# aghasemzadeh/OpenMPL

Hardware: AMD Instinct MI355X
Metric: poses/sec (V=4, J=17, batch=1024 per GPU) fp32 (higher is better)
Workload: dtype f32; 1 GPU; Human3.6M config: V=4 J=17 batch=1024 fp32, CHOSEN flag set, depth 12, DIM 32, heads 8; global_batch=1024, parallelism=single GPU

## Files before the change

openmpl_amd/csrc/spt_native.hip:

```cpp
#include <type_traits>

#include "spt_stage.hpp"

namespace mpl {

constexpr int QS = 100;
constexpr int SPT_LDS_BYTES = (ROWS * XS + ROWS * QS) * 4;

__device__ __forceinline__ int spt_abl(const SptParams& p) {
#ifdef MPL_LAB
    return p.abl;
#else
    return 0;
#endif
}

__device__ __forceinline__ void ln_frags(const float* X, int m, int li, int kq, const float4& g0, const float4& g1,
                                         const float4& b0, const float4& b1, float4& a0, float4& a1) {
    const float* xr = X + (m * 16 + li) * XS + 4 * kq;
    float4 x0 = ld4(xr), x1 = ld4(xr + 16);
    float s = ((x0.x + x0.y) + (x0.z + x0.w)) + ((x1.x + x1.y) + (x1.z + x1.w));
    s = xor16_add(s);
    s = xor32_add(s);
    const float mean = s * (1.0f / 32.0f);
    x0.x -= mean; x0.y -= mean; x0.z -= mean; x0.w -= mean;
    x1.x -= mean; x1.y -= mean; x1.z -= mean; x1.w -= mean;
    float ss = ((x0.x * x0.x + x0.y * x0.y) + (x0.z * x0.z + x0.w * x0.w)) +
               ((x1.x * x1.x + x1.y * x1.y) + (x1.z * x1.z + x1.w * x1.w));
    ss = xor16_add(ss);
    ss = xor32_add(ss);
    const float rstd = 1.0f / sqrtf(ss * (1.0f / 32.0f) + 1e-6f);
    a0.x = x0.x * rstd * g0.x + b0.x; a0.y = x0.y * rstd * g0.y + b0.y;
    a0.z = x0.z * rstd * g0.z + b0.z; a0.w = x0.w * rstd * g0.w + b0.w;
    a1.x = x1.x * rstd * g1.x + b1.x; a1.y = x1.y * rstd * g1.y + b1.y;
    a1.z = x1.z * rstd * g1.z + b1.z; a1.w = x1.w * rstd * g1.w + b1.w;
}

struct BlockFrags {
    float4 wq[6][2]; float bq[6];
    float4 wp[2][2]; float bp[2];
    float4 w1[4][2]; float b1[4];
    float4 w2[2][4]; float b2[2];
    float4 g1a, g1b, e1a, e1b;
    float4 g2a, g2b, e2a, e2b;
};

template <int N, int K>
__device__ __forceinline__ void load_tiles(const float* w, const float* b, int ldw, float4 (&wf)[N][K], float (&bf)[N], int li, int kq) {
#pragma unroll
    for (int n = 0; n < N; ++n) {
        const gfp wr = G(w) + (n * 16 + li) * ldw + 4 * kq;
#pragma unroll
        for (int q = 0; q < K; ++q) wf[n][q] = ld4(wr + 16 * q);
        bf[n] = G(b)[n * 16 + li];
    }
}
__device__ __forceinline__ void load_ln(const float* w, const float* b, float4& g0, float4& g1, float4& e0, float4& e1, int kq) {
    g0 = ld4(G(w) + 4 * kq); g1 = ld4(G(w) + 16 + 4 * kq);
    e0 = ld4(G(b) + 4 * kq); e1 = ld4(G(b) + 16 + 4 * kq);
}

constexpr int SPT_WB_VEC = 8192;
constexpr int SPT_WB_FLOATS = SPT_WB_VEC + 512;
constexpr int SPT_SMALL_ROWS = 144;
constexpr int SPT_SMALL_LDS_BYTES = (SPT_SMALL_ROWS * (XS + QS) + 2 * SPT_WB_FLOATS) * 4;
__device__ __forceinline__ const float* spt_uniform(const float* q) {
    const unsigned long long v = (unsigned long long)(uintptr_t)q;
    const unsigned lo = __builtin_amdgcn_readfirstlane((unsigned)v), hi = __builtin_amdgcn_readfirstlane((unsigned)(v >> 32));
    return reinterpret_cast<const float*>((uintptr_t)(((unsigned long long)hi << 32) | lo));
}
__device__ __forceinline__ void stage_block(const mpl_block_weights& bwv, float* wb, int wave, int lane, int w0, int nw) {
    if (wave < w0 || wave >= w0 + nw) return;
    const int li = lane & 15, kq = lane >> 4;
    struct { const float *qkv_w, *proj_w, *fc1_w, *fc2_w, *qkv_b, *proj_b, *fc1_b, *fc2_b, *ln1_w, *ln1_b, *ln2_w, *ln2_b; } bw;
    bw.qkv_w = spt_uniform(bwv.qkv_w); bw.proj_w = spt_uniform(bwv.proj_w); bw.fc1_w = spt_uniform(bwv.fc1_w); bw.fc2_w = spt_uniform(bwv.fc2_w);
    bw.qkv_b = spt_uniform(bwv.qkv_b); bw.proj_b = spt_uniform(bwv.proj_b); bw.fc1_b = spt_uniform(bwv.fc1_b); bw.fc2_b = spt_uniform(bwv.fc2_b);
    bw.ln1_w = spt_uniform(bwv.ln1_w); bw.ln1_b = spt_uniform(bwv.ln1_b); bw.ln2_w = spt_uniform(bwv.ln2_w); bw.ln2_b = spt_uniform(bwv.ln2_b);
    const unsigned lds0 = __builtin_amdgcn_readfirstlane((unsigned)(uintptr_t)(__attribute__((address_space(3))) float*)wb);
    for (int pc = wave - w0; pc < 34; pc += nw) {
        const float* src;
        bool on = true;
        if (pc < 12) src = bw.qkv_w + ((pc >> 1) * 16 + li) * SD + 16 * (pc & 1) + 4 * kq;
        else if (pc < 16) src = bw.proj_w + (((pc - 12) >> 1) * 16 + li) * SD + 16 * (pc & 1) + 4 * kq;
        else if (pc < 24) src = bw.fc1_w + (((pc - 16) >> 1) * 16 + li) * SD + 16 * (pc & 1) + 4 * kq;
        else if (pc < 32) src = bw.fc2_w + (((pc - 24) >> 2) * 16 + li) * (2 * SD) + 16 * (pc & 3) + 4 * kq;
        else if (pc == 32)
            src = lane < 24 ? bw.qkv_b + 4 * lane
                : lane < 32 ? bw.proj_b + 4 * (lane - 24)
                : lane < 48 ? bw.fc1_b + 4 * (lane - 32)
                : lane < 56 ? bw.fc2_b + 4 * (lane - 48) : bw.ln1_w + 4 * (lane - 56);
        else {
            src = lane < 8 ? bw.ln1_b + 4 * lane : lane < 16 ? bw.ln2_w + 4 * (lane - 8) : bw.ln2_b + 4 * (lane - 16);
            on = lane < 24;
        }
        if (on) dma16(src, lds0 + (unsigned)(pc * 1024));
    }
}
__device__ __forceinline__ float4 wb4(const float* wb, int piece, int lane) { return *reinterpret_cast<const float4*>(wb + piece * 256 + lane * 4); }
__device__ __forceinline__ float4 wbv4(const float* wb, int off, int kq) { return *reinterpret_cast<const float4*>(wb + SPT_WB_VEC + off + 4 * kq); }

__device__ __forceinline__ void touch(const float4& a) {
    const f32x4 v = {a.x, a.y, a.z, a.w};
    asm volatile("" ::"v"(v));
}
__device__ __forceinline__ void touch(float a) { asm volatile("" ::"v"(a)); }

__device__ __forceinline__ f32x4 tile_k32(const float4& a0, const float4& a1, const float4& w0, const float4& w1) {
    f32x4 c0 = f32x4{0.f, 0.f, 0.f, 0.f}, c1 = c0;
    c0 = mfma16(a0.x, w0.x, c0); c1 = mfma16(a1.x, w1.x, c1);
    c0 = mfma16(a0.y, w0.y, c0); c1 = mfma16(a1.y, w1.y, c1);
    c0 = mfma16(a0.z, w0.z, c0); c1 = mfma16(a1.z, w1.z, c1);
    c0 = mfma16(a0.w, w0.w, c0); c1 = mfma16(a1.w, w1.w, c1);
    return c0 + c1;
}

enum { P_QKV = 0, P_PROJ = 1, P_FC1 = 2, P_FC2 = 3 };
template <int P>
struct Phase {
    static constexpr int NT = P == P_QKV ? 6 : P == P_FC1 ? 4 : 2;
    static constexpr int KH = P == P_FC2 ? 4 : 2;
    static constexpr int PIECE = P == P_QKV ? 0 : P == P_PROJ ? 12 : P == P_FC1 ? 16 : 24;
    static constexpr int BIAS = P == P_QKV ? 0 : P == P_PROJ ? 96 : P == P_FC1 ? 128 : 192;
    static constexpr int LN = P == P_QKV ? 224 : 288;
// ... 58 lines not shown
    __device__ __forceinline__ void begin(const mpl_block_weights&, const mpl_block_weights&, bool) {}
};

template <int P, class Weights, class AFrags, class Epilogue>
__device__ __forceinline__ void linear_phase(const Weights& W, int mt, int wave, bool skip, AFrags a_frags, Epilogue epilogue) {
    constexpr int NT = Phase<P>::NT, KH = Phase<P>::KH;
    const int lo = (mt * NT * wave) / NWAVE, hi = (mt * NT * (wave + 1)) / NWAVE;
    for (int m = lo / NT; m * NT < hi && !skip; ++m) {
        float4 a[KH];
        a_frags(m, a);
#pragma unroll
        for (int n = 0; n < NT; ++n) {
            const int u = m * NT + n;
            if (u < lo || u >= hi) continue;
            float4 w[KH];
            float bias;
            W.template tile<P>(n, w, bias);
            f32x4 c = tile_k32(a[0], a[1], w[0], w[1]);
            if constexpr (KH == 4) c = c + tile_k32(a[2], a[3], w[2], w[3]);
            epilogue(m, n, c, bias);
        }
    }
}

template <bool STAGED>
__global__ __launch_bounds__(NTHR, 1) void spt_kernel(const SptParams p) {
    extern __shared__ __attribute__((aligned(1024))) float smem[];
    constexpr int RX = STAGED ? SPT_SMALL_ROWS : ROWS;
    float* WB = smem;
    float* X = smem + (STAGED ? 2 * SPT_WB_FLOATS : 0);
    float* Q = X + RX * XS;

    const int tid = threadIdx.x, lane = tid & 63, wave = __builtin_amdgcn_readfirstlane(tid >> 6);
    const int li = lane & 15, kq = lane >> 4;
    const int view = blockIdx.x % p.V;
    const int b0 = (blockIdx.x / p.V) * p.spw;
    const mpl_spt_set set = p.sets[(p.flags & MPL_F_MULTI_SPT) ? view : 0];
    const float *pose = p.poses[view], *ray = p.rays[view], *cen = p.centers[view];
    const int nl = p.B - b0 < p.spw ? p.B - b0 : p.spw;
    const int rows_live = nl * SJ;
    const int mt = (rows_live + 15) >> 4;

    std::conditional_t<STAGED, StagedWeights, FragWeights> W;
    W.li = li, W.kq = kq;
    if constexpr (STAGED) W.lane = lane;
    mpl_block_weights bw, bw_next;
    if (p.n_apps > 0) {
        bw = set.blocks[p.sched[0] & 0x7f];
        if constexpr (STAGED) stage_block(bw, WB, wave, lane, 0, NWAVE);
        else W.template load<P_QKV>(bw);
        if (STAGED && p.n_apps > 1) bw_next = set.blocks[p.sched[1] & 0x7f];
    }

    spt_embed<false>(p, set, X, tid, b0, pose, ray, cen, nl, mt * 16);
    unsigned char* sched_l = reinterpret_cast<unsigned char*>(WB + SPT_WB_FLOATS + SPT_WB_VEC + 352);
    float* conf_l = WB + SPT_WB_VEC + 352;
    if (STAGED) {
        if (tid < MPL_MAX_APPS) sched_l[tid] = p.sched[tid];
        for (int r = tid; r < rows_live; r += NTHR) {
            const int sq = r / SJ;
            conf_l[r] = pose[((size_t)(b0 + sq) * SJ + (r - sq * SJ)) * 3 + 2];
        }
        asm volatile("s_waitcnt vmcnt(0)" ::: "memory");
    }
    __syncthreads();

    const int abl = spt_abl(p);
    const bool no_mfma = (abl & 4) != 0;
    unsigned long long ph[6] = {0, 0, 0, 0, 0, 0}, tlast = (abl & 16) ? __builtin_amdgcn_s_memtime() : 0;
    auto stamp = [&](int k) {
        if (abl & 16) { const unsigned long long now = __builtin_amdgcn_s_memtime(); ph[k] += now - tlast; tlast = now; }
    };
    float4 g[2], e[2];
    auto a_ln = [&](int m, float4 (&a)[2]) { ln_frags(X, m, li, kq, g[0], g[1], e[0], e[1], a[0], a[1]); };
    auto a_q = [&](int m, auto& a) {
        const float* ar = Q + (m * 16 + li) * QS + 4 * kq;
#pragma unroll
        for (int q = 0; q < (int)(sizeof(a) / sizeof(a[0])); ++q) a[q] = ld4(ar + 16 * q);
    };
    auto add_to_x = [&](int m, int n, const f32x4& c, float b) {
        float* xd = X + (m * 16 + 4 * kq) * XS + n * 16 + li;
#pragma unroll
        for (int r = 0; r < 4; ++r) xd[r * XS] += c[r] + b;
    };
    for (int app = 0; app < p.n_apps; ++app) {
        const bool weighted = ((STAGED ? sched_l[app] : p.sched[app]) & 0x80) != 0;
        const bool more = app + 1 < p.n_apps;
        if (!STAGED && more) bw_next = set.blocks[p.sched[app + 1] & 0x7f];
        if constexpr (STAGED) W.wb = WB + (app & 1) * SPT_WB_FLOATS;
        mpl_block_weights bw_after;

        W.template begin<P_QKV>(bw, bw_next, more);
        W.template ln<P_QKV>(g, e);
        linear_phase<P_QKV>(W, mt, wave, no_mfma, a_ln, [&](int m, int n, const f32x4& c, float b) {
            float* qd = Q + (m * 16 + 4 * kq) * QS + n * 16 + li;
#pragma unroll
            for (int r = 0; r < 4; ++r) qd[r * QS] = c[r] + b;
        });
        __syncthreads();
        stamp(0);

        if (STAGED && more) {
            const int busy = (rows_live * SH + 63) >> 6;
            const int w0 = busy < NWAVE - 1 ? busy : 0;
            stage_block(bw_next, WB + ((app + 1) & 1) * SPT_WB_FLOATS, wave, lane, w0, NWAVE - w0);
            if (app + 2 < p.n_apps) bw_after = set.blocks[sched_l[app + 2] & 0x7f];
        }
// ... 19 lines not shown
            }
            float inv = 1.0f / l;
            if (weighted) {
                const int b = b0 + sq;
                if (STAGED) inv *= conf_l[r];
                else inv *= (b < p.B) ? pose[((size_t)b * SJ + (r - sq * SJ)) * 3 + 2] : 0.f;
            }
            float4 o = {0.f, 0.f, 0.f, 0.f};
#pragma unroll
            for (int j = 0; j < SJ; ++j) {
                const float4 v = ld4(kb + j * QS + SD);
                const float pj = sc[j] * inv;
                o.x = fmaf(pj, v.x, o.x);
                o.y = fmaf(pj, v.y, o.y);
                o.z = fmaf(pj, v.z, o.z);
                o.w = fmaf(pj, v.w, o.w);
            }
            st4(Q + r * QS + 4 * h, o);
        }
        __syncthreads();
        stamp(1);

        W.template begin<P_PROJ>(bw, bw_next, more);
        linear_phase<P_PROJ>(W, mt, wave, no_mfma, a_q, add_to_x);
        __syncthreads();
        stamp(2);

        W.template begin<P_FC1>(bw, bw_next, more);
        W.template ln<P_FC1>(g, e);
        linear_phase<P_FC1>(W, mt, wave, no_mfma, a_ln, [&](int m, int n, const f32x4& c, float b) {
            float* qd = Q + (m * 16 + 4 * kq) * QS + n * 16 + li;
#pragma unroll
            for (int r = 0; r < 4; ++r) qd[r * QS] = (abl & 2) ? (c[r] + b) : gelu_erf(c[r] + b);
        });
        __syncthreads();
        stamp(3);

        W.template begin<P_FC2>(bw, bw_next, more);
        linear_phase<P_FC2>(W, mt, wave, no_mfma, a_q, add_to_x);
        if (STAGED) asm volatile("s_waitcnt vmcnt(0)" ::: "memory");
        __syncthreads();
        stamp(4);
        bw = bw_next;
        if (STAGED && app + 2 < p.n_apps) bw_next = bw_after;
    }

    if (abl & 16) {
        if (lane == 0 && blockIdx.x < 32) {
            float* o = p.xs + (size_t)(blockIdx.x * NWAVE + wave) * 8;
            for (int k = 0; k < 6; ++k) o[k] = (float)ph[k];
        }
        return;
    }
    spt_epilogue<false>(p, X, tid, view, b0, pose, ray, cen, nl, rows_live);
}

int launch_spt_native(const SptParams& p, int form, int grid, hipStream_t s) {
    if (form == MPL_SPT_STAGED) {
        if (int rc = kernel_lds_once<spt_kernel<true>>(SPT_SMALL_LDS_BYTES)) return rc;
        hipLaunchKernelGGL(spt_kernel<true>, dim3(grid), dim3(NTHR), SPT_SMALL_LDS_BYTES, s, p);
    } else {
        if (int rc = kernel_lds_once<spt_kernel<false>>(SPT_LDS_BYTES)) return rc;
        hipLaunchKernelGGL(spt_kernel<false>, dim3(grid), dim3(NTHR), SPT_LDS_BYTES, s, p);
    }
    return hip_check_launch();
}

}
```

openmpl_amd/csrc/spt_packed.hip:

```cpp
#include "spt_pack.hpp"
#include "spt_stage.hpp"

namespace mpl {

constexpr int ATS = 36;
constexpr int HS = 68;
constexpr int KV_F = SJ * SH * SEQ * 4;
constexpr int SPT3_RING_BYTES = (ROWS * XS + 2 * KV_F + ROWS * ATS) * 4;
constexpr int SPT3_LDS_BYTES = 160 * 1024;
constexpr int SPT3_HID_OFF = 3072;
constexpr int SPT3_Q_OFF = 20480;
static_assert(SPT3_HID_OFF + ROWS * HS <= 2 * KV_F + ROWS * ATS, "HID does not fit its alias");
static_assert((SPT3_HID_OFF + ROWS * HS - 2 * KV_F) * 4 <= SPT3_Q_OFF, "HID reaches into the staged qkv weights");
static_assert(SPT3_Q_OFF + 12 * 1024 <= ROWS * ATS * 4, "staged qkv weights do not fit behind HID in ATT");
static_assert(SPT3_RING_BYTES + 8 * 1024 + 2 * SPT3_NPAR * 4 <= SPT3_LDS_BYTES, "spare LDS too small");

typedef float f32x2 __attribute__((ext_vector_type(2)));

__device__ inline float spt_window_scale(float v) {
    if (!(v > 0.f) || !(v < 3.0e38f)) return 1.0f;
    int e;
    (void)frexpf(32768.0f / v, &e);
    e = e - 1 < -100 ? -100 : (e - 1 > 100 ? 100 : e - 1);
    return ldexpf(1.0f, e);
}

__global__ __launch_bounds__(256) void spt_pack_kernel(const float* __restrict__ qkv_w, const float* __restrict__ qkv_b,
                                                        const float* __restrict__ ln1_w, const float* __restrict__ ln1_b,
                                                        const float* __restrict__ proj_w, const float* __restrict__ proj_b,
                                                        const float* __restrict__ fc1_w, const float* __restrict__ fc1_b,
                                                        const float* __restrict__ ln2_w, const float* __restrict__ ln2_b,
                                                        const float* __restrict__ fc2_w, const float* __restrict__ fc2_b,
                                                        char* __restrict__ dst, int fold_q) {
    __shared__ float Wf[8192];
    __shared__ float cn[SPT_NCOL], sw[SPT_NCOL], bnd[SPT_NCOL], scal[2];
    const int tid = threadIdx.x;
    for (int i = tid; i < 8192; i += 256) {
        float w;
        if (i < 3072) w = qkv_w[i] * ln1_w[i & 31];
        else if (i < 4096) w = proj_w[i - 3072];
        else if (i < 6144) w = fc1_w[i - 4096] * ln2_w[i & 31];
        else w = fc2_w[i - 6144];
        Wf[i] = w;
    }
    __syncthreads();
    if (tid < SPT_NCOL) {
        const int n = tid;
        const float *wr, *raw, *beta = nullptr;
        int K = 32;
        float bias;
        if (n < 96) { wr = Wf + n * 32; raw = qkv_w + n * 32; beta = ln1_b; bias = qkv_b[n]; }
        else if (n < 128) { wr = Wf + 3072 + (n - 96) * 32; raw = proj_w + (n - 96) * 32; bias = proj_b[n - 96]; }
        else if (n < 192) { wr = Wf + 4096 + (n - 128) * 32; raw = fc1_w + (n - 128) * 32; beta = ln2_b; bias = fc1_b[n - 128]; }
        else { wr = Wf + 6144 + (n - 192) * 64; raw = fc2_w + (n - 192) * 64; bias = fc2_b[n - 192]; K = 64; }
        float amax = 0.f;
        double ss = 0.0, c = (double)bias;
        for (int k = 0; k < K; ++k) {
            amax = fmaxf(amax, fabsf(wr[k]));
            ss += (double)wr[k] * (double)wr[k];
            if (beta) c += (double)raw[k] * (double)beta[k];
        }
        float s = 1.0f;
        if (amax > 0.f && amax < 3.0e38f) {
            int e;
            (void)frexpf(amax, &e);
            e = 14 - e;
            e = e < -100 ? -100 : (e > 100 ? 100 : e);
            s = ldexpf(1.0f, e);
// ... 136 lines not shown
#define SPT_ROLE(W, MTS, KS, LN, GELU, NCT, AST, DST, ...) \
    spt_linear_role<KS, LN, GELU, NCT, AST, DST, ((MTS) * (NCT) * (W)) / NWAVE, ((MTS) * (NCT) * ((W) + 1)) / NWAVE>(__VA_ARGS__)
#define SPT_BY_WAVE(wv, ...)                          \
    switch (wv) {                                     \
        case 0: SPT_ROLE(0, __VA_ARGS__); break;      \
        case 1: SPT_ROLE(1, __VA_ARGS__); break;      \
        case 2: SPT_ROLE(2, __VA_ARGS__); break;      \
        case 3: SPT_ROLE(3, __VA_ARGS__); break;      \
        case 4: SPT_ROLE(4, __VA_ARGS__); break;      \
        case 5: SPT_ROLE(5, __VA_ARGS__); break;      \
        case 6: SPT_ROLE(6, __VA_ARGS__); break;      \
        default: SPT_ROLE(7, __VA_ARGS__); break;     \
    }


template <int SS>
__global__ __launch_bounds__(NTHR, 1) void spt3_kernel(const SptParams p) {
    constexpr int RLIVE = SJ * SS;
    constexpr int MTS = (RLIVE + 15) / 16;
    constexpr int NT = (MTS + 3) / 4;
    extern __shared__ __attribute__((aligned(16))) float smem[];
    float* X = smem;
    float* Kb = smem + ROWS * XS;
    float* Vb = Kb + KV_F;
    float* ATT = Vb + KV_F;
    float* HID = Kb + SPT3_HID_OFF;
    char* S_W = reinterpret_cast<char*>(ATT + ROWS * ATS);
    float* S_PAR = reinterpret_cast<float*>(S_W + 8 * 1024);
    char* R_F1 = reinterpret_cast<char*>(Kb);
    char* R_Q = reinterpret_cast<char*>(ATT) + SPT3_Q_OFF;

    const int tid = threadIdx.x, lane = tid & 63;
    const int wave = __builtin_amdgcn_readfirstlane(tid >> 6);
    const int li = lane & 15, kq = lane >> 4;
    auto phase_sync = [&]() {
        asm volatile("s_waitcnt vmcnt(0)" ::: "memory");
        __syncthreads();
    };
    const int hg = wave & 1, part = wave >> 1;
    const int view = blockIdx.x % p.V;
    const int b0 = (blockIdx.x / p.V) * SS;
    const int sl = li % SS;
    const mpl_spt_set set = p.sets[(p.flags & MPL_F_MULTI_SPT) ? view : 0];
    const float* pose = p.poses[view];
    const float* ray = p.rays[view];
    const float* cen = p.centers[view];

    auto stage_w = [&](char* dst, const unsigned short* pack, int byte_off, int n_pieces) {
        const unsigned l0 = (unsigned)(uintptr_t)(__attribute__((address_space(3))) char*)dst;
        for (int i = wave; i < n_pieces; i += NWAVE)
            ::mpl::dma16(reinterpret_cast<const float*>(reinterpret_cast<const char*>(pack) + byte_off + i * 1024) + lane * 4,
                         l0 + (unsigned)(i * 1024));
    };
    auto load_par = [&](const mpl_block_weights& b) -> float4 {
        if (tid >= SPT3_NPAR / 4) return float4{0.f, 0.f, 0.f, 0.f};
        return ld4(G(reinterpret_cast<const float*>(reinterpret_cast<const char*>(b.qkv_w3) + SPT_PACK_VEC)) + 4 * tid);
    };
    auto store_par = [&](int app_of, const float4& v) {
        if (tid < SPT3_NPAR / 4) st4(S_PAR + (app_of & 1) * SPT3_NPAR + 4 * tid, v);
    };
    mpl_block_weights bw;
    if (p.n_apps > 0) {
        bw = set.blocks[p.sched[0] & 0x7f];
        stage_w(R_Q, bw.qkv_w3, SPT_PACK_QKV, 12);
    }
    const float4 par0 = p.n_apps > 0 ? load_par(bw) : float4{0.f, 0.f, 0.f, 0.f};
    spt_embed<true, SS>(p, set, X, tid, b0, pose, ray, cen, SS, MTS * 16);
    store_par(0, par0);
    phase_sync();

    auto load_w = [&](const char* region, int unit, sf16x8 (&w)[2]) { spt_load_unit(region, unit, lane, w); };
    auto ln_frag = [&](int m, sf16x8& ah, sf16x8& al) {
        const float* xr = X + (m * 16 + li) * XS + 8 * kq;
        spt_ln_split(::mpl::ld4(xr), ::mpl::ld4(xr + 4), ah, al);
    };
    for (int app = 0; app < p.n_apps; ++app) {
        const bool weighted = (p.sched[app] & 0x80) != 0;
        bw = set.blocks[p.sched[app] & 0x7f];
        const unsigned short* pack = bw.qkv_w3;
        const float* par = S_PAR + (app & 1) * SPT3_NPAR;
        stage_w(S_W, pack, SPT_PACK_PROJ, 4);
        {
            sf16x8 wq[3][2];
            float4 bq[3], sq[3];
#pragma unroll
            for (int c = 0; c < 3; ++c) {
                load_w(R_Q, 2 * c + hg, wq[c]);
                bq[c] = ::mpl::ld4(par + SPT_C_QKV + 32 * c + 16 * hg + 4 * kq);
                sq[c] = ::mpl::ld4(par + SPT_NCOL + SPT_C_QKV + 32 * c + 16 * hg + 4 * kq);
            }
            float4 q[NT];
#pragma unroll
            for (int t = 0; t < NT; ++t) {
                q[t] = float4{0.f, 0.f, 0.f, 0.f};
                if (part + 4 * t < MTS && !(p.abl & 8)) {
                    const int m = part + 4 * t;
                    const int j = (16 * m + li) / SS;
                    const bool live = 16 * m + li < RLIVE;
                    sf16x8 ah, al;
                    ln_frag(m, ah, al);
                    const f32x4 z = {0.f, 0.f, 0.f, 0.f};
                    const f32x4 cq = mfma3(wq[0], ah, al, z), ck = mfma3(wq[1], ah, al, z), cv = mfma3(wq[2], ah, al, z);
                    q[t] = float4{fmaf(cq[0], sq[0].x, bq[0].x), fmaf(cq[1], sq[0].y, bq[0].y), fmaf(cq[2], sq[0].z, bq[0].z),
                                  fmaf(cq[3], sq[0].w, bq[0].w)};
                    const int h = 4 * hg + kq;
                    const float kx = fmaf(ck[0], sq[1].x, bq[1].x), ky = fmaf(ck[1], sq[1].y, bq[1].y);
                    const float kz = fmaf(ck[2], sq[1].z, bq[1].z), kw = fmaf(ck[3], sq[1].w, bq[1].w);
                    if (live && j < SJ - 1) {
                        float* kp = Kb + ((((j >> 1) * 2) * SH + h) * SS + sl) * 4 + (j & 1);
                        kp[0] = kx;
                        kp[2] = ky;
                        kp[SH * SS * 4] = kz;
                        kp[SH * SS * 4 + 2] = kw;
                    } else if (live) {
                        st4(Kb + (SJ - 1) * SH * SS * 4 + (h * SS + sl) * 4, float4{kx, ky, kz, kw});
                    }
                    if (live)
                        st4(Vb + ((j * SH + h) * SS + sl) * 4, float4{fmaf(cv[0], sq[2].x, bq[2].x), fmaf(cv[1], sq[2].y, bq[2].y),
                                                                       fmaf(cv[2], sq[2].z, bq[2].z), fmaf(cv[3], sq[2].w, bq[2].w)});
                }
// ... 55 lines not shown
                for (int t = 0; t < NL; ++t) o[t] = float4{0.f, 0.f, 0.f, 0.f};
#pragma unroll
                for (int j = 0; j < SJ; ++j) {
                    const float4 v = ::mpl::ld4(Vb + ((j * SH + h) * SS + sl) * 4);
#pragma unroll
                    for (int t = 0; t < NL; ++t) {
                        const float pj = sc[t][j];
                        o[t].x = fmaf(pj, v.x, o[t].x);
                        o[t].y = fmaf(pj, v.y, o[t].y);
                        o[t].z = fmaf(pj, v.z, o[t].z);
                        o[t].w = fmaf(pj, v.w, o[t].w);
                    }
                }
#pragma unroll
                for (int t = 0; t < NL; ++t) {
                    o[t] = float4{o[t].x * inv[t], o[t].y * inv[t], o[t].z * inv[t], o[t].w * inv[t]};
                    if (weighted) {
                        const float big = fmaxf(fmaxf(fabsf(o[t].x), fabsf(o[t].y)), fmaxf(fabsf(o[t].z), fabsf(o[t].w)));
                        if (!(big <= 65000.f)) {
                            const float qn = __builtin_nanf("");
                            o[t] = float4{qn, qn, qn, qn};
                            if (p.err_host) __hip_atomic_fetch_or(p.err_host, 2u, __ATOMIC_RELAXED, __HIP_MEMORY_SCOPE_SYSTEM);
                        }
                    }
                }
#pragma unroll
                for (int t = 0; t < NL; ++t) st4(ATT + ((part + 4 * t) * 16 + li) * ATS + 4 * h, o[t]);
            };
            if (!(p.abl & 1)) {
                if (part + 4 * (NT - 1) < MTS) attention(SptInt<NT>{});
                else if (NT > 1) attention(SptInt<(NT > 1 ? NT - 1 : 1)>{});
            }
        }
        phase_sync();
        stage_w(R_F1, pack, SPT_PACK_FC1, 8);
        if (!(p.abl & 32)) SPT_BY_WAVE(wave, MTS, 1, false, false, 2, ATS, XS, ATT, X, S_W, par, SPT_C_PROJ, 0.f, lane);
        phase_sync();
        stage_w(S_W, pack, SPT_PACK_FC2, 8);
        if (!(p.abl & 64))
            SPT_BY_WAVE(wave, MTS, 1, true, true, 4, XS, HS, X, HID, R_F1, par, SPT_C_FC1, par[2 * SPT_NCOL + 1], lane);
        phase_sync();
        {
            float4 parn = float4{0.f, 0.f, 0.f, 0.f};
            if (app + 1 < p.n_apps) {
                const mpl_block_weights bn = set.blocks[p.sched[app + 1] & 0x7f];
                stage_w(R_Q, bn.qkv_w3, SPT_PACK_QKV, 12);
                parn = load_par(bn);
            }
            if (!(p.abl & 128)) SPT_BY_WAVE(wave, MTS, 2, false, false, 2, HS, XS, HID, X, S_W, par, SPT_C_FC2, 0.f, lane);
            if (app + 1 < p.n_apps) store_par(app + 1, parn);
        }
        phase_sync();
    }
    spt_epilogue<true, SS>(p, X, tid, view, b0, pose, ray, cen, SS, MTS * 16);
}

template <int SS>
static int launch_spt3(const SptParams& p, int grid, hipStream_t s) {
    if (int rc = kernel_lds_once<spt3_kernel<SS>>(SPT3_LDS_BYTES)) return rc;
    hipLaunchKernelGGL(spt3_kernel<SS>, dim3(grid), dim3(NTHR), SPT3_LDS_BYTES, s, p);
    return hip_check_launch();
}

int launch_spt_packed(const SptParams& p, int ss, int grid, hipStream_t s) {
    switch (ss) {
        case 1: return launch_spt3<1>(p, grid, s);
        case 2: return launch_spt3<2>(p, grid, s);
        case 4: return launch_spt3<4>(p, grid, s);
        case 8: return launch_spt3<8>(p, grid, s);
        case 16: return launch_spt3<16>(p, grid, s);
        default: return MPL_E_INVALID;
    }
}

}
```

openmpl_amd/csrc/spt_stage.hpp:

```cpp
#pragma once
#include "common.hpp"

namespace mpl {

constexpr int SJ = 17;
constexpr int SD = 32;
constexpr int SH = 8;
constexpr int SEQ = 16;
constexpr int ROWS = SEQ * SJ;
constexpr int XS = 36;
constexpr int NTHR = 512;
constexpr int NWAVE = NTHR / 64;
constexpr int SPT_SMALL_SPW = 8;

struct SptParams {
    const float* poses[MPL_MAX_VIEWS];
    const float* rays[MPL_MAX_VIEWS];
    const float* centers[MPL_MAX_VIEWS];
    const mpl_spt_set* sets;
    const float *snorm_w, *snorm_b;
    const float *pos3d_embed, *pos3d_view, *pos3d_lin_w, *pos3d_lin_b;
    const float *ray_w, *ray_b, *cfpt_w, *cfpt_b;
    float* xs;
    int B, V, in_ch, n_apps;
    unsigned flags;
    int c3;
    int spw;
    int abl;
    unsigned* err_host;
    unsigned char sched[MPL_MAX_APPS];
};

int launch_spt_native(const SptParams& p, int form, int grid, hipStream_t s);
int launch_spt_packed(const SptParams& p, int ss, int grid, hipStream_t s);

typedef const __attribute__((address_space(1))) float* gfp;
__device__ __forceinline__ gfp G(const float* p) { return (gfp)p; }
__device__ __forceinline__ float4 ld4(gfp p) {
    typedef float v4 __attribute__((ext_vector_type(4)));
    const v4 t = *reinterpret_cast<const __attribute__((address_space(1))) v4*>(p);
    return make_float4(t.x, t.y, t.z, t.w);
}

template <bool TM, int SS = SEQ>
__device__ __forceinline__ void row_to_sj(int r, int& sq, int& j) {
    if (TM) { j = r / SS; sq = r % SS; }
    else { sq = r / SJ; j = r - sq * SJ; }
}

template <bool TM, int SS = SEQ>
__device__ __forceinline__ void spt_embed(const SptParams& p, const mpl_spt_set& set, float* X, int tid, int b0,
                                          const float* pose, const float* ray, const float* cen, int nseq = SEQ, int nrows = ROWS) {
    for (int idx = tid; idx < nrows * SD; idx += NTHR) {
        const int r = idx >> 5, c = idx & 31;
        int sq, j;
        row_to_sj<TM, SS>(r, sq, j);
        const int b = b0 + sq;
        float x = 0.f;
        if (b < p.B && sq < nseq && j < SJ) {
            const float* in = pose + ((size_t)b * SJ + j) * 3;
            const float* we = set.embed_w + c * p.in_ch;
            x = set.embed_b[c] + we[0] * in[0] + we[1] * in[1];
            if (p.in_ch == 3) x += we[2] * in[2];
            if (p.flags & MPL_F_CONF_ADD) x += set.conf_w[c] * in[2] + set.conf_b[c];
            if (p.flags & MPL_F_CONF_MULT) x *= set.conf_w[c] * in[2] + set.conf_b[c];
            x += set.pos_embed[j * SD + c];
            if (p.flags & MPL_F_POS3D_SPATIAL) {
                if (p.flags & MPL_F_POS3D_LEARN) {
                    x += p.pos3d_embed[j * p.c3 + c];
                } else {
                    const float* rr = ray + ((size_t)b * SJ + j) * 3;
                    const float* cc = cen + (size_t)b * 3;
                    const float vx = rr[0] - cc[0], vy = rr[1] - cc[1], vz = rr[2] - cc[2];
                    const float nrm = fmaxf(sqrtf(vx * vx + vy * vy + vz * vz), 1e-12f);
                    const float* wl = p.pos3d_lin_w + c * 3;
                    x += p.pos3d_lin_b[c] + wl[0] * (vx / nrm) + wl[1] * (vy / nrm) + wl[2] * (vz / nrm);
                }
            }
        }
        X[r * XS + c] = x;
    }
}

template <bool TM, int SS = SEQ>
__device__ __forceinline__ void spt_epilogue(const SptParams& p, const float* X, int tid, int view, int b0, const float* pose,
                                             const float* ray, const float* cen, int nseq = SEQ, int nrows = ROWS) {
    const bool to_rays = (p.flags & MPL_F_POS3D_TO_RAYS) && (p.flags & MPL_F_RAYS_TOKEN);
    const bool ray_tok = !(p.flags & MPL_F_POS3D_TO_RAYS) && (p.flags & MPL_F_RAYS_TOKEN);
    const int cw = to_rays ? 2 * SD : SD;
    const int Df = SJ * SD * ((p.flags & MPL_F_RAYS_TOKEN) ? 2 : 1);
    for (int r = tid; r < nrows; r += NTHR) {
        int sq, j;
        row_to_sj<TM, SS>(r, sq, j);
        const int b = b0 + sq;
        if (b >= p.B || sq >= nseq || j >= SJ) continue;
        const float* xr = X + r * XS;
        float v[SD];
        float s = 0.f;
#pragma unroll
        for (int c = 0; c < SD; c += 4) {
            const float4 t = ld4(xr + c);
            v[c] = t.x; v[c + 1] = t.y; v[c + 2] = t.z; v[c + 3] = t.w;
            s += (t.x + t.y) + (t.z + t.w);
        }
        const float mean = s * (1.0f / 32.0f);
        float ss = 0.f;
#pragma unroll
        for (int c = 0; c < SD; ++c) {
            v[c] -= mean;
            ss = fmaf(v[c], v[c], ss);
        }
        const float rstd = 1.0f / sqrtf(ss * (1.0f / 32.0f) + 1e-6f);
        const float conf = pose[((size_t)b * SJ + j) * 3 + 2];
        float dx = 0.f, dy = 0.f, dz = 0.f, nx = 0.f, ny = 0.f, nz = 0.f;
        const bool need_dir = (p.flags & MPL_F_RAYS_TOKEN) ||
                              (!(p.flags & MPL_F_POS3D_SPATIAL) && !(p.flags & MPL_F_POS3D_LEARN));
        if (need_dir) {
            const float* rr = ray + ((size_t)b * SJ + j) * 3;
            const float* cc = cen + (size_t)b * 3;
            dx = rr[0] - cc[0]; dy = rr[1] - cc[1]; dz = rr[2] - cc[2];
            const float nrm = fmaxf(sqrtf(dx * dx + dy * dy + dz * dz), 1e-12f);
            nx = dx / nrm; ny = dy / nrm; nz = dz / nrm;
        }
        auto pos3d = [=](int c) -> float {
            if (p.flags & MPL_F_POS3D_SPATIAL) return p.pos3d_view[j * p.c3 + c];
            if (p.flags & MPL_F_POS3D_LEARN) return p.pos3d_embed[j * p.c3 + c];
            const float* wl = p.pos3d_lin_w + c * 3;
            return p.pos3d_lin_b[c] + wl[0] * nx + wl[1] * ny + wl[2] * nz;
        };
        auto ray_emb = [=](int c) -> float {
            const float* wr = p.ray_w + c * 3;
            return p.ray_b[c] + wr[0] * dx + wr[1] * dy + wr[2] * dz;
        };
        float* orow = p.xs + ((size_t)b * p.V + view) * Df;
        float* o1 = orow + j * cw;
#pragma unroll
        for (int c = 0; c < SD; c += 4) {
            float t[4];
#pragma unroll
            for (int q = 0; q < 4; ++q) {
                float y = v[c + q] * rstd * p.snorm_w[c + q] + p.snorm_b[c + q];
                if (p.flags & MPL_F_CONF_IN_FPT) y += p.cfpt_w[c + q] * conf + p.cfpt_b[c + q];
                t[q] = y + pos3d(c + q);
            }
            st4(o1 + c, float4{t[0], t[1], t[2], t[3]});
        }
        if (to_rays) {
#pragma unroll
            for (int c = 0; c < SD; c += 4) {
                float t[4];
#pragma unroll
                for (int q = 0; q < 4; ++q) t[q] = ray_emb(c + q) + pos3d(SD + c + q);
                st4(o1 + SD + c, float4{t[0], t[1], t[2], t[3]});
            }
        } else if (ray_tok) {
            float* o2 = orow + (SJ + j) * SD;
#pragma unroll
            for (int c = 0; c < SD; c += 4) st4(o2 + c, float4{ray_emb(c), ray_emb(c + 1), ray_emb(c + 2), ray_emb(c + 3)});
        }
    }
}

}
```

Measured before the change: 851,100 poses/s.

## Stage embedding and epilogue operands into LDS via DMA and restructure both ends

Before the embedding and the final norm/output epilogue, pose, ray, center and small parameter vectors are copied into LDS with global_load_lds DMA spread across waves. The embedding then reads these from LDS using a per-thread fixed-column layout with flag-specialised passes. The epilogue first computes per-row statistics into LDS, then writes output as coalesced float4 stores indexed by output position instead of per-row serial stores. This removes scattered global reads and uncoalesced writes at the kernel ends, at the cost of extra barriers, LDS aliasing constraints and more code paths.

New measurement: 858,300 poses/s (median of 6 runs). Within noise of the previous version (+0.8%).

```diff
diff --git a/openmpl_amd/csrc/spt_native.hip b/openmpl_amd/csrc/spt_native.hip
--- a/openmpl_amd/csrc/spt_native.hip
+++ b/openmpl_amd/csrc/spt_native.hip
@@ -6,6 +6,8 @@
 
 constexpr int QS = 100;
 constexpr int SPT_LDS_BYTES = (ROWS * XS + ROWS * QS) * 4;
+constexpr int SPT_Q_STATS = 3072;
+static_assert(SE_FLOATS <= 144 * QS && SO_FLOATS <= SPT_Q_STATS && SPT_Q_STATS + ST_FLOATS <= 144 * QS, "the staged operands of the ends do not fit Q");
 
 __device__ __forceinline__ int spt_abl(const SptParams& p) {
 #ifdef MPL_LAB
@@ -64,11 +66,6 @@
 constexpr int SPT_WB_FLOATS = SPT_WB_VEC + 512;
 constexpr int SPT_SMALL_ROWS = 144;
 constexpr int SPT_SMALL_LDS_BYTES = (SPT_SMALL_ROWS * (XS + QS) + 2 * SPT_WB_FLOATS) * 4;
-__device__ __forceinline__ const float* spt_uniform(const float* q) {
-    const unsigned long long v = (unsigned long long)(uintptr_t)q;
-    const unsigned lo = __builtin_amdgcn_readfirstlane((unsigned)v), hi = __builtin_amdgcn_readfirstlane((unsigned)(v >> 32));
-    return reinterpret_cast<const float*>((uintptr_t)(((unsigned long long)hi << 32) | lo));
-}
 __device__ __forceinline__ void stage_block(const mpl_block_weights& bwv, float* wb, int wave, int lane, int w0, int nw) {
     if (wave < w0 || wave >= w0 + nw) return;
     const int li = lane & 15, kq = lane >> 4;
@@ -233,7 +230,10 @@
         if (STAGED && p.n_apps > 1) bw_next = set.blocks[p.sched[1] & 0x7f];
     }
 
-    spt_embed<false>(p, set, X, tid, b0, pose, ray, cen, nl, mt * 16);
+    spt_stage_embed(p, set, Q, wave, lane, b0, nl, pose, ray, cen);
+    asm volatile("s_waitcnt vmcnt(0)" ::: "memory");
+    __syncthreads();
+    spt_embed<false, SEQ, RX * SD / NTHR>(p, X, Q, tid, b0, nl, mt * 16);
     unsigned char* sched_l = reinterpret_cast<unsigned char*>(WB + SPT_WB_FLOATS + SPT_WB_VEC + 352);
     float* conf_l = WB + SPT_WB_VEC + 352;
     if (STAGED) {
@@ -359,7 +359,17 @@
         }
         return;
     }
-    spt_epilogue<false>(p, X, tid, view, b0, pose, ray, cen, nl, rows_live);
+    {
+        const int l = (int)__builtin_amdgcn_mbcnt_hi(~0u, __builtin_amdgcn_mbcnt_lo(~0u, 0u));
+        int w = wave, bb = __builtin_amdgcn_readfirstlane(b0);
+        asm volatile("" : "+s"(w), "+s"(bb));
+        const SptParams& pp = spt_params_here(p);
+        const int nlive = pp.B - bb < pp.spw ? pp.B - bb : pp.spw;
+        spt_stage_epilogue(pp, Q, w, l, bb, nlive, pp.poses[view], pp.rays[view], pp.centers[view]);
+        asm volatile("s_waitcnt vmcnt(0)" ::: "memory");
+        __syncthreads();
+        spt_epilogue<false>(pp, X, Q, Q + SPT_Q_STATS, w * 64 + l, view, bb, nlive, nlive * SJ);
+    }
 }
 
 int launch_spt_native(const SptParams& p, int form, int grid, hipStream_t s) {
diff --git a/openmpl_amd/csrc/spt_packed.hip b/openmpl_amd/csrc/spt_packed.hip
--- a/openmpl_amd/csrc/spt_packed.hip
+++ b/openmpl_amd/csrc/spt_packed.hip
@@ -14,6 +14,9 @@
 static_assert((SPT3_HID_OFF + ROWS * HS - 2 * KV_F) * 4 <= SPT3_Q_OFF, "HID reaches into the staged qkv weights");
 static_assert(SPT3_Q_OFF + 12 * 1024 <= ROWS * ATS * 4, "staged qkv weights do not fit behind HID in ATT");
 static_assert(SPT3_RING_BYTES + 8 * 1024 + 2 * SPT3_NPAR * 4 <= SPT3_LDS_BYTES, "spare LDS too small");
+static_assert(SE_FLOATS <= KV_F, "the staged embedding operands reach beyond K");
+static_assert(SO_FLOATS * 4 <= 12 * 1024, "the staged epilogue operands do not fit the 12 KiB of the qkv weights");
+static_assert(ST_FLOATS <= KV_F, "the epilogue's row statistics reach beyond K");
 
 typedef float f32x2 __attribute__((ext_vector_type(2)));
 
@@ -256,12 +259,14 @@
             ::mpl::dma16(reinterpret_cast<const float*>(reinterpret_cast<const char*>(pack) + byte_off + i * 1024) + lane * 4,
                          l0 + (unsigned)(i * 1024));
     };
+    static_assert(SPT3_NPAR / 4 > 64 && SPT3_NPAR / 4 <= 128, "the parameter vectors are one float4 of the first two waves");
+    auto par_thread = [&]() { return wave == 0 || (wave == 1 && lane < SPT3_NPAR / 4 - 64); };
     auto load_par = [&](const mpl_block_weights& b) -> float4 {
-        if (tid >= SPT3_NPAR / 4) return float4{0.f, 0.f, 0.f, 0.f};
-        return ld4(G(reinterpret_cast<const float*>(reinterpret_cast<const char*>(b.qkv_w3) + SPT_PACK_VEC)) + 4 * tid);
+        if (!par_thread()) return float4{0.f, 0.f, 0.f, 0.f};
+        return ld4(G(reinterpret_cast<const float*>(reinterpret_cast<const char*>(b.qkv_w3) + SPT_PACK_VEC)) + 256 * wave + 4 * lane);
     };
     auto store_par = [&](int app_of, const float4& v) {
-        if (tid < SPT3_NPAR / 4) st4(S_PAR + (app_of & 1) * SPT3_NPAR + 4 * tid, v);
+        if (par_thread()) st4(S_PAR + (app_of & 1) * SPT3_NPAR + 256 * wave + 4 * lane, v);
     };
     mpl_block_weights bw;
     if (p.n_apps > 0) {
@@ -269,7 +274,17 @@
         stage_w(R_Q, bw.qkv_w3, SPT_PACK_QKV, 12);
     }
     const float4 par0 = p.n_apps > 0 ? load_par(bw) : float4{0.f, 0.f, 0.f, 0.f};
-    spt_embed<true, SS>(p, set, X, tid, b0, pose, ray, cen, SS, MTS * 16);
+    const bool ends = !(p.abl & 256);
+    if (ends) {
+        const int nlive = p.B - b0 < SS ? p.B - b0 : SS;
+        spt_stage_embed(p, set, Kb, wave, lane, b0, nlive, pose, ray, cen);
+    }
+    phase_sync();
+    if (ends) {
+        int t = tid;
+        asm volatile("" : "+v"(t));
+        spt_embed<true, SS, MTS>(p, X, Kb, t, b0, SS, MTS * 16);
+    }
     store_par(0, par0);
     phase_sync();
 
@@ -431,7 +446,16 @@
         }
         phase_sync();
     }
-    spt_epilogue<true, SS>(p, X, tid, view, b0, pose, ray, cen, SS, MTS * 16);
+    if (!(p.abl & 256)) {
+        const int l = (int)__builtin_amdgcn_mbcnt_hi(~0u, __builtin_amdgcn_mbcnt_lo(~0u, 0u));
+        int bb = b0;
+        asm volatile("" : "+s"(bb));
+        const SptParams& pp = spt_params_here(p);
+        float* E = reinterpret_cast<float*>(R_Q);
+        spt_stage_epilogue(pp, E, wave, l, bb, pp.B - bb < SS ? pp.B - bb : SS, pp.poses[view], pp.rays[view], pp.centers[view]);
+        phase_sync();
+        spt_epilogue<true, SS>(pp, X, E, Kb, wave * 64 + l, view, bb, SS, MTS * 16);
+    }
 }
 
 template <int SS>
diff --git a/openmpl_amd/csrc/spt_stage.hpp b/openmpl_amd/csrc/spt_stage.hpp
--- a/openmpl_amd/csrc/spt_stage.hpp
+++ b/openmpl_amd/csrc/spt_stage.hpp
@@ -1,4 +1,6 @@
 #pragma once
+#include <type_traits>
+
 #include "common.hpp"
 
 namespace mpl {
@@ -48,52 +50,190 @@
     else { sq = r / SJ; j = r - sq * SJ; }
 }
 
+constexpr int SE_W = 0, SE_B = 96, SE_CW = 128, SE_CB = 160, SE_POS = 192;
+constexpr int SE_P3 = SE_POS + SJ * SD;
+constexpr int SP_P3_FLOATS = SJ * 2 * SD, SP_LINB = 3 * 2 * SD;
+constexpr int SE_POSE = SE_P3 + SP_P3_FLOATS, SE_RAY = SE_POSE + ROWS * 3, SE_CEN = SE_RAY + ROWS * 3;
+constexpr int SE_FLOATS = SE_CEN + SEQ * 3;
+constexpr int SO_NW = 0, SO_NB = 32, SO_CW = 64, SO_CB = 96, SO_RW = 128, SO_RB = 224;
+constexpr int SO_P3 = 256;
+constexpr int SO_POSE = SO_P3 + SP_P3_FLOATS, SO_RAY = SO_POSE + ROWS * 3, SO_CEN = SO_RAY + ROWS * 3;
+constexpr int SO_FLOATS = SO_CEN + SEQ * 3;
+constexpr int ST_S = 9;
+constexpr int ST_FLOATS = ROWS * ST_S;
+static_assert(SP_LINB + 2 * SD <= SP_P3_FLOATS, "the linear 3D encoding does not fit the slot of the table");
+
+__device__ __forceinline__ const float* spt_uniform(const float* q) {
+    const unsigned long long v = (unsigned long long)(uintptr_t)q;
+    const unsigned lo = __builtin_amdgcn_readfirstlane((unsigned)v), hi = __builtin_amdgcn_readfirstlane((unsigned)(v >> 32));
+    return reinterpret_cast<const float*>((uintptr_t)(((unsigned long long)hi << 32) | lo));
+}
+__device__ __forceinline__ void dma4(const float* g, unsigned lds_dst) {
+    unsigned keep;
+    asm volatile(
+        "s_mov_b32 %0, m0\n\t"
+        "s_mov_b32 m0, %2\n\t"
+        "s_nop 0\n\t"
+        "global_load_lds_dword %1, off\n\t"
+        "s_mov_b32 m0, %0"
+        : "=&s"(keep)
+        : "v"(g), "s"(lds_dst)
+        : "memory");
+}
+__device__ __forceinline__ const SptParams& spt_params_here(const SptParams& p) {
+    typedef const __attribute__((address_space(4))) char* kptr;
+    unsigned off = 0;
+    asm volatile("" : "+s"(off));
+    return *(const SptParams*)(const char*)((kptr)(const char*)&p + off);
+}
+__device__ __forceinline__ void spt_stage_vec(float* dst, const float* src, int n, int wave, int lane, int rot) {
+    src = spt_uniform(src);
+    const unsigned l0 = __builtin_amdgcn_readfirstlane((unsigned)(uintptr_t)dst);
+    for (int k = (wave - rot) & (NWAVE - 1); k * 64 < n; k += NWAVE)
+        if (k * 64 + lane < n) dma4(src + k * 64 + lane, l0 + (unsigned)(k * 256));
+}
+__device__ __forceinline__ void spt_stage_inputs(float* E, int o_pose, int o_ray, int o_cen, bool dirs, int b0, int nlive,
+                                                 const float* pose, const float* ray, const float* cen, int wave, int lane) {
+    spt_stage_vec(E + o_pose, pose + (size_t)b0 * SJ * 3, nlive * SJ * 3, wave, lane, 0);
+    if (dirs) {
+        spt_stage_vec(E + o_ray, ray + (size_t)b0 * SJ * 3, nlive * SJ * 3, wave, lane, 5);
+        spt_stage_vec(E + o_cen, cen + (size_t)b0 * 3, nlive * 3, wave, lane, 2);
+    }
+}
+__device__ __forceinline__ void spt_stage_embed(const SptParams& p, const mpl_spt_set& set, float* E, int wave, int lane, int b0,
+                                                int nlive, const float* pose, const float* ray, const float* cen) {
+    const bool lin = (p.flags & MPL_F_POS3D_SPATIAL) && !(p.flags & MPL_F_POS3D_LEARN);
+    spt_stage_inputs(E, SE_POSE, SE_RAY, SE_CEN, lin, b0, nlive, pose, ray, cen, wave, lane);
+    spt_stage_vec(E + SE_POS, set.pos_embed, SJ * SD, wave, lane, 3);
+    spt_stage_vec(E + SE_W, set.embed_w, SD * p.in_ch, wave, lane, 4);
+    spt_stage_vec(E + SE_B, set.embed_b, SD, wave, lane, 6);
+    if (p.flags & (MPL_F_CONF_ADD | MPL_F_CONF_MULT)) {
+        spt_stage_vec(E + SE_CW, set.conf_w, SD, wave, lane, 7);
+        spt_stage_vec(E + SE_CB, set.conf_b, SD, wave, lane, 1);
+    }
+    if (lin) {
+        spt_stage_vec(E + SE_P3, p.pos3d_lin_w, 3 * p.c3, wave, lane, 1);
+        spt_stage_vec(E + SE_P3 + SP_LINB, p.pos3d_lin_b, p.c3, wave, lane, 7);
+    } else if (p.flags & MPL_F_POS3D_SPATIAL) {
+        spt_stage_vec(E + SE_P3, p.pos3d_embed, SJ * p.c3, wave, lane, 1);
+    }
+}
+__device__ __forceinline__ void spt_stage_epilogue(const SptParams& p, float* E, int wave, int lane, int b0, int nlive,
+                                                   const float* pose, const float* ray, const float* cen) {
+    const bool table = (p.flags & (MPL_F_POS3D_SPATIAL | MPL_F_POS3D_LEARN)) != 0;
+    spt_stage_inputs(E, SO_POSE, SO_RAY, SO_CEN, (p.flags & MPL_F_RAYS_TOKEN) || !table, b0, nlive, pose, ray, cen, wave, lane);
+    spt_stage_vec(E + SO_NW, p.snorm_w, SD, wave, lane, 3);
+    spt_stage_vec(E + SO_NB, p.snorm_b, SD, wave, lane, 4);
+    if (p.flags & MPL_F_CONF_IN_FPT) {
+        spt_stage_vec(E + SO_CW, p.cfpt_w, SD, wave, lane, 6);
+        spt_stage_vec(E + SO_CB, p.cfpt_b, SD, wave, lane, 7);
+    }
+    if (p.flags & MPL_F_RAYS_TOKEN) {
+        spt_stage_vec(E + SO_RW, p.ray_w, 3 * SD, wave, lane, 6);
+        spt_stage_vec(E + SO_RB, p.ray_b, SD, wave, lane, 7);
+    }
+    if (table) {
+        spt_stage_vec(E + SO_P3, (p.flags & MPL_F_POS3D_SPATIAL) ? p.pos3d_view : p.pos3d_embed, SJ * p.c3, wave, lane, 1);
+    } else {
+        spt_stage_vec(E + SO_P3, p.pos3d_lin_w, 3 * p.c3, wave, lane, 1);
+        spt_stage_vec(E + SO_P3 + SP_LINB, p.pos3d_lin_b, p.c3, wave, lane, 4);
+    }
+}
+
+__device__ __forceinline__ float spt_lin3(const float* w, float b, float x, float y, float z) {
+#pragma clang fp contract(off)
+    return (fmaf(w[0], x, b) + w[1] * y) + w[2] * z;
+}
+__device__ __forceinline__ float spt_ray3(const float* w, float b, float x, float y, float z) {
+    return fmaf(w[2], z, fmaf(w[1], y, fmaf(w[0], x, b)));
+}
+__device__ __forceinline__ void spt_dir(const float* rr, const float* cc, float (&d)[3], float (&n)[3]) {
+#pragma clang fp contract(off)
+    d[0] = rr[0] - cc[0]; d[1] = rr[1] - cc[1]; d[2] = rr[2] - cc[2];
+    const float nrm = fmaxf(sqrtf(fmaf(d[0], d[0], d[1] * d[1]) + d[2] * d[2]), 1e-12f);
+    n[0] = d[0] / nrm; n[1] = d[1] / nrm; n[2] = d[2] / nrm;
+}
+
+template <bool TM, int SS = SEQ, int NTRIP = ROWS * SD / NTHR>
+__device__ __forceinline__ void spt_embed(const SptParams& p, float* X, const float* E, int tid, int b0, int nseq = SEQ, int nrows = ROWS) {
+#pragma clang fp contract(off)
+    const int c = tid & 31, r0 = tid >> 5;
+    auto row = [&](int k, int& a, int& j) -> bool {
+        int sq;
+        row_to_sj<TM, SS>(r0 + 16 * k, sq, j);
+        const bool live = b0 + sq < p.B && sq < nseq && j < SJ;
+        j = live ? j : 0;
+        a = live ? sq * SJ + j : 0;
+        return live;
+    };
+    float* xc = X + r0 * XS + c;
+    const float eb = E[SE_B + c], w0 = E[SE_W + c * p.in_ch], w1 = E[SE_W + c * p.in_ch + 1];
+    auto first = [&](int a) { return (eb + w0 * E[SE_POSE + 3 * a]) + w1 * E[SE_POSE + 3 * a + 1]; };
+    const bool extra = p.in_ch == 3 || (p.flags & (MPL_F_CONF_ADD | MPL_F_CONF_MULT));
+    if (extra) {
+#pragma unroll
+        for (int k = 0; k < NTRIP; ++k) {
+            int a, j;
+            row(k, a, j);
+            if (r0 + 16 * k < nrows) xc[k * 16 * XS] = first(a);
+        }
+        auto pass = [&](auto f) {
+#pragma unroll
+            for (int k = 0; k < NTRIP; ++k) {
+                int a, j;
+                row(k, a, j);
+                if (r0 + 16 * k < nrows) xc[k * 16 * XS] = f(xc[k * 16 * XS], E[SE_POSE + 3 * a + 2]);
+            }
+        };
+        if (p.in_ch == 3) {
+            const float w2 = E[SE_W + c * 3 + 2];
+            pass([&](float x, float conf) { return fmaf(w2, conf, x); });
+        }
+        const float cw = E[SE_CW + c], cb = E[SE_CB + c];
+        if (p.flags & MPL_F_CONF_ADD) pass([&](float x, float conf) { return x + fmaf(cw, conf, cb); });
+        if (p.flags & MPL_F_CONF_MULT) pass([&](float x, float conf) { return x * fmaf(cw, conf, cb); });
+    }
+    auto last = [&](auto from_x, auto mode) {
+#pragma unroll
+        for (int k = 0; k < NTRIP; ++k) {
+            int a, j;
+            const bool live = row(k, a, j);
+            float x = decltype(from_x)::value ? xc[k * 16 * XS] : first(a);
+            x = x + E[SE_POS + j * SD + c];
+            if constexpr (decltype(mode)::value == 1) x = x + E[SE_P3 + j * p.c3 + c];
+            if constexpr (decltype(mode)::value == 2) {
+                float d[3], n[3];
+                spt_dir(E + SE_RAY + 3 * a, E + SE_CEN + 3 * (a / SJ), d, n);
+                x = x + spt_lin3(E + SE_P3 + 3 * c, E[SE_P3 + SP_LINB + c], n[0], n[1], n[2]);
+            }
+            if (r0 + 16 * k < nrows) xc[k * 16 * XS] = live ? x : 0.f;
+        }
+    };
+    constexpr std::true_type yes{};
+    constexpr std::false_type no{};
+    constexpr std::integral_constant<int, 0> m0{};
+    constexpr std::integral_constant<int, 1> m1{};
+    constexpr std::integral_constant<int, 2> m2{};
+    const int mode = !(p.flags & MPL_F_POS3D_SPATIAL) ? 0 : (p.flags & MPL_F_POS3D_LEARN) ? 1 : 2;
+    if (extra) { if (mode == 0) last(yes, m0); else if (mode == 1) last(yes, m1); else last(yes, m2); }
+    else { if (mode == 0) last(no, m0); else if (mode == 1) last(no, m1); else last(no, m2); }
+}
+
 template <bool TM, int SS = SEQ>
-__device__ __forceinline__ void spt_embed(const SptParams& p, const mpl_spt_set& set, float* X, int tid, int b0,
-                                          const float* pose, const float* ray, const float* cen, int nseq = SEQ, int nrows = ROWS) {
-    for (int idx = tid; idx < nrows * SD; idx += NTHR) {
-        const int r = idx >> 5, c = idx & 31;
-        int sq, j;
-        row_to_sj<TM, SS>(r, sq, j);
-        const int b = b0 + sq;
-        float x = 0.f;
-        if (b < p.B && sq < nseq && j < SJ) {
-            const float* in = pose + ((size_t)b * SJ + j) * 3;
-            const float* we = set.embed_w + c * p.in_ch;
-            x = set.embed_b[c] + we[0] * in[0] + we[1] * in[1];
-            if (p.in_ch == 3) x += we[2] * in[2];
-            if (p.flags & MPL_F_CONF_ADD) x += set.conf_w[c] * in[2] + set.conf_b[c];
-            if (p.flags & MPL_F_CONF_MULT) x *= set.conf_w[c] * in[2] + set.conf_b[c];
-            x += set.pos_embed[j * SD + c];
-            if (p.flags & MPL_F_POS3D_SPATIAL) {
-                if (p.flags & MPL_F_POS3D_LEARN) {
-                    x += p.pos3d_embed[j * p.c3 + c];
-                } else {
-                    const float* rr = ray + ((size_t)b * SJ + j) * 3;
-                    const float* cc = cen + (size_t)b * 3;
-                    const float vx = rr[0] - cc[0], vy = rr[1] - cc[1], vz = rr[2] - cc[2];
-                    const float nrm = fmaxf(sqrtf(vx * vx + vy * vy + vz * vz), 1e-12f);
-                    const float* wl = p.pos3d_lin_w + c * 3;
-                    x += p.pos3d_lin_b[c] + wl[0] * (vx / nrm) + wl[1] * (vy / nrm) + wl[2] * (vz / nrm);
-                }
-            }
-        }
-        X[r * XS + c] = x;
-    }
-}
-
-template <bool TM, int SS = SEQ>
-__device__ __forceinline__ void spt_epilogue(const SptParams& p, const float* X, int tid, int view, int b0, const float* pose,
-                                             const float* ray, const float* cen, int nseq = SEQ, int nrows = ROWS) {
+__device__ __forceinline__ void spt_epilogue(const SptParams& p, const float* X, const float* E, float* ST, int tid, int view, int b0,
+                                             int nseq = SEQ, int nrows = ROWS) {
+#pragma clang fp contract(off)
     const bool to_rays = (p.flags & MPL_F_POS3D_TO_RAYS) && (p.flags & MPL_F_RAYS_TOKEN);
     const bool ray_tok = !(p.flags & MPL_F_POS3D_TO_RAYS) && (p.flags & MPL_F_RAYS_TOKEN);
     const int cw = to_rays ? 2 * SD : SD;
     const int Df = SJ * SD * ((p.flags & MPL_F_RAYS_TOKEN) ? 2 : 1);
+    const bool table = (p.flags & (MPL_F_POS3D_SPATIAL | MPL_F_POS3D_LEARN)) != 0;
+    const bool need_dir = (p.flags & MPL_F_RAYS_TOKEN) || !table;
+    const int nlive = p.B - b0 < nseq ? p.B - b0 : nseq;
     for (int r = tid; r < nrows; r += NTHR) {
         int sq, j;
         row_to_sj<TM, SS>(r, sq, j);
-        const int b = b0 + sq;
-        if (b >= p.B || sq >= nseq || j >= SJ) continue;
+        if (sq >= nlive || j >= SJ) continue;
         const float* xr = X + r * XS;
         float v[SD];
         float s = 0.f;
@@ -103,62 +243,73 @@
             v[c] = t.x; v[c + 1] = t.y; v[c + 2] = t.z; v[c + 3] = t.w;
             s += (t.x + t.y) + (t.z + t.w);
         }
-        const float mean = s * (1.0f / 32.0f);
         float ss = 0.f;
 #pragma unroll
         for (int c = 0; c < SD; ++c) {
-            v[c] -= mean;
+            v[c] = fmaf(s, -1.0f / 32.0f, v[c]);
             ss = fmaf(v[c], v[c], ss);
         }
-        const float rstd = 1.0f / sqrtf(ss * (1.0f / 32.0f) + 1e-6f);
-        const float conf = pose[((size_t)b * SJ + j) * 3 + 2];
-        float dx = 0.f, dy = 0.f, dz = 0.f, nx = 0.f, ny = 0.f, nz = 0.f;
-        const bool need_dir = (p.flags & MPL_F_RAYS_TOKEN) ||
-                              (!(p.flags & MPL_F_POS3D_SPATIAL) && !(p.flags & MPL_F_POS3D_LEARN));
+        float* st = ST + r * ST_S;
+        st[0] = s;
+        st[1] = 1.0f / sqrtf(fmaf(ss, 1.0f / 32.0f, 1e-6f));
+        st[2] = E[SO_POSE + 3 * (sq * SJ + j) + 2];
         if (need_dir) {
-            const float* rr = ray + ((size_t)b * SJ + j) * 3;
-            const float* cc = cen + (size_t)b * 3;
-            dx = rr[0] - cc[0]; dy = rr[1] - cc[1]; dz = rr[2] - cc[2];
-            const float nrm = fmaxf(sqrtf(dx * dx + dy * dy + dz * dz), 1e-12f);
-            nx = dx / nrm; ny = dy / nrm; nz = dz / nrm;
-        }
-        auto pos3d = [=](int c) -> float {
-            if (p.flags & MPL_F_POS3D_SPATIAL) return p.pos3d_view[j * p.c3 + c];
-            if (p.flags & MPL_F_POS3D_LEARN) return p.pos3d_embed[j * p.c3 + c];
-            const float* wl = p.pos3d_lin_w + c * 3;
-            return p.pos3d_lin_b[c] + wl[0] * nx + wl[1] * ny + wl[2] * nz;
-        };
-        auto ray_emb = [=](int c) -> float {
-            const float* wr = p.ray_w + c * 3;
-            return p.ray_b[c] + wr[0] * dx + wr[1] * dy + wr[2] * dz;
-        };
-        float* orow = p.xs + ((size_t)b * p.V + view) * Df;
-        float* o1 = orow + j * cw;
-#pragma unroll
-        for (int c = 0; c < SD; c += 4) {
+            float d[3], n[3];
+            spt_dir(E + SO_RAY + 3 * (sq * SJ + j), E + SO_CEN + 3 * sq, d, n);
+            st[3] = d[0]; st[4] = d[1]; st[5] = d[2];
+            st[6] = n[0]; st[7] = n[1]; st[8] = n[2];
+        }
+    }
+    __syncthreads();
+    const int n4 = nlive * (SJ * SD / 4);
+    auto where = [&](int i, int& sq, int& j, int& c) {
+        sq = i / (SJ * SD / 4);
+        const int rem = i - sq * (SJ * SD / 4);
+        j = rem >> 3;
+        c = (rem & 7) * 4;
+        return TM ? j * SS + sq : sq * SJ + j;
+    };
+    auto out_row = [&](int sq) { return p.xs + ((size_t)(b0 + sq) * p.V + view) * Df; };
+    auto pos3d = [&](auto lin, const float* st, int j, int c) -> float {
+        if constexpr (decltype(lin)::value) return spt_lin3(E + SO_P3 + 3 * c, E[SO_P3 + SP_LINB + c], st[6], st[7], st[8]);
+        else return E[SO_P3 + j * p.c3 + c];
+    };
+    auto main_run = [&](auto cfpt, auto lin) {
+        for (int i = tid; i < n4; i += NTHR) {
+            int sq, j, c;
+            const int r = where(i, sq, j, c);
+            const float4 xv = ld4(X + r * XS + c);
+            const float* st = ST + r * ST_S;
+            const float xq[4] = {xv.x, xv.y, xv.z, xv.w};
             float t[4];
 #pragma unroll
             for (int q = 0; q < 4; ++q) {
-                float y = v[c + q] * rstd * p.snorm_w[c + q] + p.snorm_b[c + q];
-                if (p.flags & MPL_F_CONF_IN_FPT) y += p.cfpt_w[c + q] * conf + p.cfpt_b[c + q];
-                t[q] = y + pos3d(c + q);
+                float y = fmaf(fmaf(st[0], -1.0f / 32.0f, xq[q]) * st[1], E[SO_NW + c + q], E[SO_NB + c + q]);
+                if constexpr (decltype(cfpt)::value) y = y + fmaf(E[SO_CW + c + q], st[2], E[SO_CB + c + q]);
+                t[q] = y + pos3d(lin, st, j, c + q);
             }
-            st4(o1 + c, float4{t[0], t[1], t[2], t[3]});
-        }
-        if (to_rays) {
-#pragma unroll
-            for (int c = 0; c < SD; c += 4) {
-                float t[4];
-#pragma unroll
-                for (int q = 0; q < 4; ++q) t[q] = ray_emb(c + q) + pos3d(SD + c + q);
-                st4(o1 + SD + c, float4{t[0], t[1], t[2], t[3]});
+            st4(out_row(sq) + j * cw + c, float4{t[0], t[1], t[2], t[3]});
+        }
+    };
+    auto ray_run = [&](auto beside, auto lin) {
+        for (int i = tid; i < n4; i += NTHR) {
+            int sq, j, c;
+            const float* st = ST + where(i, sq, j, c) * ST_S;
+            float t[4];
+#pragma unroll
+            for (int q = 0; q < 4; ++q) {
+                t[q] = spt_ray3(E + SO_RW + 3 * (c + q), E[SO_RB + c + q], st[3], st[4], st[5]);
+                if constexpr (decltype(beside)::value) t[q] = t[q] + pos3d(lin, st, j, SD + c + q);
             }
-        } else if (ray_tok) {
-            float* o2 = orow + (SJ + j) * SD;
-#pragma unroll
-            for (int c = 0; c < SD; c += 4) st4(o2 + c, float4{ray_emb(c), ray_emb(c + 1), ray_emb(c + 2), ray_emb(c + 3)});
-        }
-    }
-}
-
-}
+            st4(out_row(sq) + (decltype(beside)::value ? j * cw + SD : (SJ + j) * SD) + c, float4{t[0], t[1], t[2], t[3]});
+        }
+    };
+    constexpr std::true_type yes{};
+    constexpr std::false_type no{};
+    if (p.flags & MPL_F_CONF_IN_FPT) { if (table) main_run(yes, no); else main_run(yes, yes); }
+    else { if (table) main_run(no, no); else main_run(no, yes); }
+    if (to_rays) { if (table) ray_run(yes, no); else ray_run(yes, yes); }
+    else if (ray_tok) ray_run(no, no);
+}
+
+}
```
